# JuliaQuantumControl/GRAPE.jl

Measured on AMD Instinct MI355X. Metric: GRAPE gradient evals/sec (N=64, 1000 steps, 128 traj), higher is better.
Workload: dtype f64

## Files before the change

### grape.jl_amd/api.py

```python
from __future__ import annotations

import ctypes as C
import os
import subprocess
import sys

import numpy as np

_HERE = os.path.dirname(os.path.abspath(__file__))
_CSRC = os.path.join(_HERE, "csrc")
_LIBNAME = "libgrape_hip.so"

J_T_SM, J_T_SS, J_T_RE = 0, 1, 2
GRAD_GRADGEN, GRAD_TAYLOR = 0, 1
PROP_EXP, PROP_SERIES = 0, 1
ABI_VERSION = 7

STATUS = {0: "GRAPE_OK", -1: "GRAPE_ERR_INVALID", -2: "GRAPE_ERR_HIP", -3: "GRAPE_ERR_CHI_NORM",
          -4: "GRAPE_ERR_SINGULAR", -5: "GRAPE_ERR_TAYLOR", -6: "GRAPE_ERR_NO_CONTROLS", -7: "GRAPE_ERR_AGAIN",
          -8: "GRAPE_ERR_HOST"}

EXPORTS = ["grape_create", "grape_destroy", "grape_eval", "grape_forward", "grape_backward",
           "grape_forward_device", "grape_backward_device", "grape_check", "grape_get_propagator",
           "grape_get_tau_grads", "grape_get_storage", "grape_get_timings", "grape_reset_timings", "grape_get_work",
           "grape_last_error", "grape_abi_version", "grape_set_fused_sweeps", "grape_get_sums", "grape_backward_xi",
           "grape_get_final_states", "grape_backward_chi",
           "grape_get_time_gradient", "grape_set_tlist", "grape_eval_batch", "grape_get_batch_info", "grape_create_open",
           "grape_hvp", "grape_get_hvp_info", "grape_open_time_gradient", "grape_open_hvp", "grape_get_open_hvp_info",
           "grape_open_eval_batch", "grape_get_open_batch_info", "grape_open_set_running_cost", "grape_open_backward_xi"]


class GrapeHipError(RuntimeError):
    def __init__(self, code, msg):
        super().__init__(f"{STATUS.get(code, code)}: {msg}")
        self.code = code


class _Problem(C.Structure):
    _fields_ = [("abi_version", C.c_int32), ("N", C.c_int32), ("L", C.c_int32), ("K", C.c_int32),
# ... 39 lines not shown
                'grape_asm_co_start:\n\t.incbin "grape_asm.co"\ngrape_asm_co_end:\n\t.byte 0\n'
                '\t.section .note.GNU-stack,"",@progbits\n')
    cmds.append(["gcc", "-c", "-fPIC", "asm_embed.S", "-o", "asm_embed.o"])
    for c in cmds:
        res = subprocess.run(c, capture_output=True, text=True, cwd=work)
        if verbose or res.returncode:
            print(" ".join(c), res.stdout, res.stderr)
        if res.returncode:
            raise RuntimeError("assembling the gfx950 kernels failed")
    return emb_o


def _sources():
    srcs = [os.path.join(_CSRC, f) for f in ("grape_hip.hip", "grape_t18.hip", "grape_kernels.hip.h", "grape_large.hip.h",
                                             "grape_series.hip.h", "grape_cheby.hip.h", "grape_t18.hip.h", "grape_t18_coeffs.h",
                                             "grape_deriv3.hip.h", "grape_timegrad.hip.h", "grape_batch.hip.h", "grape_lindblad.hip.h", "grape_lindblad_tg.hip.h", "grape_hvp.hip.h", "grape_lindblad_hvp.hip.h", "grape_lindblad_batch.hip.h", "grape_lindblad_rc.hip.h", "grape_devmem.h", os.path.join("asm", "gen_t16.py"), os.path.join("asm", "gen_t16p.py"), os.path.join("asm", "gen_t18g.py"), os.path.join("asm", "gen_t18gp.py"), os.path.join("asm", "gen_d3.py"), os.path.join("asm", "gen_d3s.py"), os.path.join("asm", "gen_lg.py"), os.path.join("asm", "gen_d4.py"), os.path.join("asm", "gcn.py"))]
    return srcs, os.path.join(_HERE, "..", "include", "grape_hip.h")


def _up_to_date(out: str) -> bool:
    srcs, hdr = _sources()
    return os.path.exists(out) and all(os.path.getmtime(out) >= os.path.getmtime(s) for s in srcs + [hdr])


def build_library(force: bool = False, verbose: bool = False, extra_flags=(), out: str | None = None) -> str:
    import fcntl
    import shutil
    import tempfile
    out = out or library_path()
    if not force and _up_to_date(out):
        return out
# ... 55 lines not shown
    lib.grape_create.argtypes = [C.POINTER(vp), C.POINTER(_Problem)]
    lib.grape_create_open.argtypes = [C.POINTER(vp), C.POINTER(_Problem), C.POINTER(_Lindblad)]
    lib.grape_destroy.argtypes = [vp]
    lib.grape_destroy.restype = None
    lib.grape_eval.argtypes = [vp, vp, dp, vp, vp, vp]
    lib.grape_forward.argtypes = [vp, vp, vp]
    lib.grape_backward.argtypes = [vp, vp, vp]
    lib.grape_forward_device.argtypes = [vp, vp, vp, vp]
    lib.grape_backward_device.argtypes = [vp, vp, vp, vp]
    lib.grape_check.argtypes = [vp, vp]
    lib.grape_get_propagator.argtypes = [vp, ip, ip, vp]
    lib.grape_get_tau_grads.argtypes = [vp, vp]
    lib.grape_get_storage.argtypes = [vp, ip, vp]
    lib.grape_get_timings.argtypes = [vp, vp, ip]
    lib.grape_get_work.argtypes = [vp, vp, ip]
    lib.grape_reset_timings.argtypes = [vp]
    lib.grape_set_fused_sweeps.argtypes = [vp, ip]
    lib.grape_get_sums.argtypes = [vp, vp]
    lib.grape_get_final_states.argtypes = [vp, vp]
    lib.grape_backward_chi.argtypes = [vp, vp, vp]
    lib.grape_backward_xi.argtypes = [vp, vp, vp, vp, C.c_double, vp]
    lib.grape_get_time_gradient.argtypes = [vp, vp]
    lib.grape_open_time_gradient.argtypes = [vp, vp]
    lib.grape_set_tlist.argtypes = [vp, vp]
    lib.grape_eval_batch.argtypes = [vp, ip, vp, vp, vp, vp]
    lib.grape_get_batch_info.argtypes = [vp, vp, ip]
    lib.grape_hvp.argtypes = [vp, ip, vp, vp]
    lib.grape_get_hvp_info.argtypes = [vp, vp, ip]
    lib.grape_open_hvp.argtypes = [vp, ip, vp, vp]
    lib.grape_get_open_hvp_info.argtypes = [vp, vp, ip]
# ... 236 lines not shown

    def timings(self):
        ms = np.full(8, -1.0)
        self._lib.grape_get_timings(self._h, ms.ctypes.data, 8)
        out = dict(zip(["expm", "forward", "backward", "deriv", "reduce", "total"], ms[:6].tolist()))
        if ms[6] >= 0.0:
            out["host_enqueue"] = float(ms[6])
        if ms[7] >= 0.0:
            out["gradient_allreduce_us"] = float(ms[7]) * 1e3
        return out

    def reset_timings(self):
        self._chk(self._lib.grape_reset_timings(self._h))

    def work(self):
        w = np.zeros(19)
        self._lib.grape_get_work(self._h, w.ctypes.data, 19)
        return dict(cells=w[0], squarings=w[1], flop_expm=w[2], flop_deriv=w[3], deriv_orders=w[4],
                    pivoted_cells=w[5], expm_cells=w[6], series_terms=w[7], series_steps=w[8],
                    t18_mfma_flop=w[9], t18_squarings=w[10], t18_cells=w[11], matrix_free_fallback=w[12], t16_cells=w[13],
                    asm_kernel=w[14], asm_deriv_kernel=w[15], asm_blocked_products=w[16],
                    walk_steps=w[17], scan_block=w[18])


def liouvillian(H, cops=()):
    H = np.asarray(H, dtype=np.complex128)
    d = H.shape[0]
    if H.shape != (d, d):
        raise ValueError(f"H must be [d, d], got {H.shape}")
    eye = np.eye(d)
    heff = H.copy()
    for A in cops:
        A = np.asarray(A, dtype=np.complex128)
        heff = heff - 0.5j * (A.conj().T @ A)
    out = np.kron(eye, heff) - np.kron(heff.conj(), eye)
    for A in cops:
        A = np.asarray(A, dtype=np.complex128)
# ... 172 lines not shown
```

### grape.jl_amd/csrc/asm/gen_t16.py

```python
import os
import re
import struct
import sys

sys.path.insert(0, os.path.dirname(os.path.abspath(__file__)))
from gcn import Prog, Reg, V, A, S, VCC, EXEC, Neg, Abs, kernel_text

NT = 4
NP = 64
LDB = (3 * NP + 2) * 8
PLB = NP * 8
TROW = 16 * LDB
PLANES = NP * LDB
E1 = PLANES
EXH = 256 * 8 + 128
EXW = 2 * EXH
E2 = E1 + 4 * EXW
RED = E2 + 4 * EXW
XS0 = RED + 16 * 8
XS1 = XS0 + 1024
LDS_BYTES = XS1 + 1024
KERNARG = 136

HERE = os.path.dirname(os.path.abspath(__file__))


def t16_coeffs():
    txt = open(os.path.join(HERE, "..", "grape_t18_coeffs.h")).read()
    c = {}
    for m in re.finditer(r"#define\s+T16_(C\d+|THETA)\s+([-+0-9.eE]+)", txt):
        c[m.group(1)] = float(m.group(2))
    assert len(c) == 17, c
    return c


def dbits(x):
    b = struct.unpack("<Q", struct.pack("<d", x))[0]
# ... 335 lines not shown
        p.salu("s_lshl_b32", t0, t1, 16)
        p.salu("s_lshr_b32", t1, t1, 16)
        p.salu("s_add_u32", self.s_sb.sub(0), self.s_Sf.sub(0), t0)
        p.salu("s_addc_u32", self.s_sb.sub(1), self.s_Sf.sub(1), t1)

    def cell_bases_finish(self, kc):
        p = self.p
        t0, t1 = self.s_tmp[0], self.s_tmp[1]
        p.s_waitcnt(lgkm=0)
        p.s_cmp("s_cmp_lg_u64", self.s_rep, 0)
        p.salu("s_cselect_b32", self.s_k, self.s_k, kc)
        p.salu("s_lshl_b32", t0, self.s_k, 16)
        p.salu("s_lshr_b32", t1, self.s_k, 16)
        p.salu("s_add_u32", self.s_hb.sub(0), self.s_H0.sub(0), t0)
        p.salu("s_addc_u32", self.s_hb.sub(1), self.s_H0.sub(1), t1)
        p.salu("s_lshl_b32", t0, self.s_snext, 20)
        p.salu("s_sub_u32", self.s_dt.sub(1), self.s_dt.sub(1), t0)

    def cell_bases(self, kc, n, cell):
        self.cell_bases_issue(kc, n, cell)
        self.cell_bases_finish(kc)

    def fetch(self, u, dst, half=None):
        p = self.p
        (i0, j0), (i1, j1) = TILES[2 * u], TILES[2 * u + 1]
        toff = self.s_tmp[2]
        p.s_cmp("s_cmp_lt_u32", self.s_wave, 2)
        self.ssel(toff, (16 * i0 * NP + 16 * j0) * 8, (16 * i1 * NP + 16 * j1) * 8)
        if half in (None, 0):
            p.salu("s_add_u32", self.s_t0.sub(0), self.s_hb.sub(0), toff)
            p.salu("s_addc_u32", self.s_t0.sub(1), self.s_hb.sub(1), 0)
# ... 292 lines not shown
                streams.append([lambda xr=xr, ar_=ar_: self.acc_read(xr, ar_),
                                lambda xi=xi, ai_=ai_: self.acc_read(xi, ai_),
                                lambda xr=xr: p.valu("v_mul_f64", xr, c[2], xr),
                                lambda xi=xi: p.valu("v_mul_f64", xi, c[2], xi),
                                lambda xr=xr, a2r=a2r: p.valu("v_fma_f64", xr, c[1], a2r, xr),
                                lambda xi=xi, a2i=a2i: p.valu("v_fma_f64", xi, c[1], a2i, xi),
                                lambda xs=xs, xr=xr, xi=xi: p.valu("v_add_f64", xs, xr, xi),
                                lambda r=r, a2r=a2r, a2i=a2i: p.valu("v_add_f64", A2sm[sl].d(r), a2r, a2i)])
            self.interleave(streams)

        self.product(Qt, [A2re, A2im, A2sm], fused={"valu": valu2, "stores": lambda sl: self.plane_stores(sl, tt[0], tt[1], Qt[sl][1])})
        for t in tt + A2sm:
            vp.free(t)
        self.cell_bases_finish(self.s_nkc)
        self.stamp(3)
        facc, gacc, cacc = vp.alloc(), vp.alloc(), vp.alloc()
        for acc in (facc, gacc, cacc):
            for j in range(8):
                p.valu("v_mov_b32", acc.sub(j), 0)
        streams = []
        for sl in range(4):
            for r in range(4):
                k = len(streams) % 4
                p1, p2, p3 = (Qt[sl][j].d(r) for j in range(3))
                a2r, a2i = A2re[sl].d(r), A2im[sl].d(r)
                f, g_, cs = facc.d(k), gacc.d(k), cacc.d(k)
                streams.append([
                    lambda p3=p3, p1=p1: p.valu("v_add_f64", p3, p3, Neg(p1)),
                    lambda p1=p1, p2=p2: p.valu("v_add_f64", p1, p1, Neg(p2)),
                    lambda p3=p3, p2=p2: p.valu("v_add_f64", p3, p3, Neg(p2)),
# ... 2 lines not shown
                    lambda g_=g_, a2r=a2r, p1=p1: p.valu("v_fma_f64", g_, a2r, p1, g_),
                    lambda cs=cs, a2i=a2i: p.valu("v_add_f64", cs, cs, Abs(a2i)),
                    lambda f=f, p3=p3: p.valu("v_fma_f64", f, p3, p3, f),
                    lambda g_=g_, a2i=a2i, p3=p3: p.valu("v_fma_f64", g_, a2i, p3, g_)])
        for g in range(0, 16, 4):
            self.interleave(streams[g:g + 4])
        f, g_, cs = facc.d(0), gacc.d(0), cacc.d(0)
        for k in range(1, 4):
            p.valu("v_add_f64", f, f, facc.d(k))
            p.valu("v_add_f64", g_, g_, gacc.d(k))
            p.valu("v_add_f64", cs, cs, cacc.d(k))
        ones, ct = cacc.d(1), vp.alloc(1)
        lo, hi = dbits(1.0)
        p.valu("v_mov_b32", ones.sub(0), lo)
        p.valu("v_mov_b32", ones.sub(1), hi)
        p.mfma(ct, ones, cs, 0)
        tmp = cacc.d(2)
        self.wave_reduce(f, tmp, "v_add_f64")
        self.wave_reduce(g_, tmp, "v_add_f64")
        mx = cacc.d(3)
        p.valu("v_mov_b64", mx, ct.d(0))
        for ctrl in ("quad_perm:[1,0,3,2]", "quad_perm:[2,3,0,1]", "row_half_mirror", "row_mirror"):
            p.dpp_mov(tmp.sub(0), mx.sub(0), ctrl)
            p.dpp_mov(tmp.sub(1), mx.sub(1), ctrl)
            p.valu("v_max_f64", mx, mx, tmp)
        vrd = ct.sub(2)
        p.salu("s_lshl_b32", self.s_tmp[0], self.s_wave, 3)
        p.salu("s_add_u32", self.s_tmp[0], self.s_tmp[0], RED)
        p.valu("v_mov_b32", vrd, self.s_tmp[0])
        p.salu("s_mov_b64", self.s_save, EXEC)
        self.set_exec(0, 0x80000000)
# ... 37 lines not shown
        p.s_cmp("s_cmp_eq_u64", S(58, 2), 0)
        p.salu("s_cselect_b32", self.s_tmp[4], 2, 0)
        p.salu("s_or_b32", self.s_prop, self.s_prop, self.s_tmp[4])
        p.valu("v_cndmask_b32", vz.sub(1), 1, 0, S(58, 2))
        p.salu("s_lshl_b32", self.s_tmp[2], self.s_cell, 2)
        p.valu("v_mov_b32", vz.sub(2), self.s_tmp[2])
        p.salu("s_mov_b64", self.s_save, EXEC)
        p.s_cmp("s_cmp_eq_u32", self.s_wave, 0)
        p.salu("s_cselect_b32", self.s_tmp[4], 1, 0)
        p.salu("s_mov_b32", self.s_tmp[5], 0)
        p.salu("s_mov_b64", EXEC, S(self.s_tmp[4].idx, 2))
        p.global_store(1, vz.sub(2), vz.sub(1), self.s_verdict)
        p.salu("s_mov_b64", EXEC, self.s_save)
        for t in (vtf, vtg, vt2, vz):
            vp.free(t)
        self.A2p_re, self.A2p_im = ap.alloc(4), ap.alloc(4)
        Bre, Bim, Bsm = [None] * 4, [None] * 4, [None] * 4
        tt = [vp.alloc(), vp.alloc()]

        def valu3(sl):
            Bre[sl], Bim[sl], Bsm[sl] = vp.alloc(), vp.alloc(), vp.alloc()
            streams = []
            for r in range(4):
                y0r, xs, y0i = (Qt[sl][j].d(r) for j in range(3))
                a2r, a2i = A2re[sl].d(r), A2im[sl].d(r)
                xr, xi = tt[0].d(r), tt[1].d(r)
                br, bi, bs = Bre[sl].d(r), Bim[sl].d(r), Bsm[sl].d(r)
                ar_, ai_ = A_(sl, r)
                pr, pi_ = self.A2p_re.sub(8 * sl, 8).d(r), self.A2p_im.sub(8 * sl, 8).d(r)
                streams.append([
# ... 101 lines not shown
                            "after_first": lambda: bsm([0]), "post": post4})
        for t in tt:
            vp.free(t)
        if not self.early_free:
            ap.free(self.A2p_re)
            ap.free(self.A2p_im)
        for t in Bre + Bim + Bsm:
            vp.free(t)
        self.stamp(9)
        if not self.early_free:
            ap.free(self.As_re)
            ap.free(self.As_im)
        Un = vp.alloc(8, at=self.UT)
        uid = len(p.ins)
        L_sq, L_sq_loop, L_res = f"L_sq_{uid}", f"L_sq_loop_{uid}", f"L_res_{uid}"
        p.s_cmp("s_cmp_lg_u32", self.s_scur, 0)
        p.s_branch("s_cbranch_scc1", L_sq)
        streams = []
        for sl in range(4):
            for r in range(4):
                p1, p2, p3 = (Qt[sl][j].d(r) for j in range(3))
                ur, ui = Un.sub(16 * sl + 4 * r, 2), Un.sub(16 * sl + 4 * r + 2, 2)
                streams.append([lambda ur=ur, p1=p1, p2=p2: p.valu("v_add_f64", ur, p1, Neg(p2)),
                                lambda ui=ui, p3=p3, p1=p1: p.valu("v_add_f64", ui, p3, Neg(p1)),
                                lambda ui=ui, p2=p2: p.valu("v_add_f64", ui, ui, Neg(p2))])
        for g in range(0, 16, 4):
            self.interleave(streams[g:g + 4])
        p.s_barrier()
        p.s_branch("s_branch", L_res)
        p.label(L_sq)
        vp.free(Un)
        in_place_y(range(4))
        p.s_barrier()
        p.salu("s_mov_b32", self.s_sqc, self.s_scur)
        p.label(L_sq_loop)
        Q2 = [[vp.alloc() for _ in range(3)] for _ in range(4)]

        def valu_sq(sl):
            for r in range(4):
                p.valu("v_add_f64", Qt[sl][1].d(r), Qt[sl][0].d(r), Qt[sl][2].d(r))

        self.product(Q2, [[Qt[sl][0] for sl in range(4)], [Qt[sl][2] for sl in range(4)], [Qt[sl][1] for sl in range(4)]],
                     fused={"valu": valu_sq, "stores": lambda sl: self.plane_stores(sl, Qt[sl][0], Qt[sl][2], Qt[sl][1])})
        streams = []
        for sl in range(4):
            for r in range(4):
                q1, q2, q3 = (Q2[sl][j].d(r) for j in range(3))
                tr, ti = Qt[sl][0].d(r), Qt[sl][2].d(r)
                streams.append([lambda tr=tr, q1=q1, q2=q2: p.valu("v_add_f64", tr, q1, Neg(q2)),
# ... 315 lines not shown
```

### grape.jl_amd/csrc/grape_hip.hip

```cpp
#include "../../include/grape_hip.h"
#include "grape_kernels.hip.h"
#include "grape_t18_coeffs.h"
#include "grape_econ_coeffs.h"
#include "grape_large.hip.h"
#include "grape_series.hip.h"
#include "grape_cheby.hip.h"
#include "grape_timegrad.hip.h"
#include "grape_lindblad.hip.h"
#include "grape_lindblad_tg.hip.h"
#include "grape_hvp.hip.h"
#include "grape_lindblad_hvp.hip.h"
#include "grape_lindblad_batch.hip.h"
#include "grape_lindblad_rc.hip.h"
#include "grape_devmem.h"

#include <rccl/rccl.h>
#include <dlfcn.h>
#include <mutex>

#include <algorithm>
#include <chrono>
#include <cmath>
#include <cstdio>
#include <cstdlib>
#include <cstring>
#include <new>
#include <stdexcept>
#include <string>
#include <thread>
// ... 63 lines not shown
    double *d_eps = nullptr;
    double2 *d_U = nullptr, *d_fw = nullptr, *d_bw = nullptr, *d_tg = nullptr;
    double *d_ret = nullptr;
    double *d_out = nullptr;
    double *d_f = nullptr, *d_G = nullptr, *d_rho = nullptr;
    int *d_flags = nullptr;
    int *d_cellflag = nullptr;
    int KC = 0;
    bool herm = false;
    bool herm_ctrl = false;
    bool t18 = false;
    bool t18_small = true;
    bool t16 = true;
    double *d_gram = nullptr;
    int *d_celllist = nullptr;
    bool asm16 = false;
    bool asm16p = false;
    double *d_dte = nullptr;
    bool asm18gp = false;
    bool asm18g = false;
    int *d_wgtab = nullptr, *d_prog = nullptr, *d_splan = nullptr;
    double2 *d_xinit = nullptr;
    int asm_blocks = 0;
    int last_walk_fuse = 0;
    bool asm_sq = true;
    int asm_walk = 0;
    bool foreign_stream = false;
    bool credit_pending = false;
    std::vector<double> bal;
    std::vector<double> bal_stage_chi, bal_stage_xi;
// ... 2520 lines not shown
                    gram[(size_t)kc * GS + (size_t)a * M + b] = gram[(size_t)kc * GS + (size_t)b * M + a] = sum;
                }
        }
        if (!p->hc_per_traj)
            for (int l = 0; l < L; ++l) kap_shared[l] = shape_factor(p->Hc + (size_t)l * nn2, gram[(size_t)(1 + l) * M + (1 + l)]);
        parallel_for(KCn, [&](int kc) {
            const int k = repk[kc] < 0 ? kc : repk[kc];
            for (int a = 0; a < M; ++a) {
                const double fro2 = gram[(size_t)kc * GS + (size_t)a * M + a];
                const double *o = a == 0 ? p->H0 + (size_t)k * nn2 : p->Hc + ((size_t)(p->hc_per_traj ? k : 0) * L + (a - 1)) * nn2;
                gram[(size_t)kc * GS + (size_t)M * M + a] = (a > 0 && !p->hc_per_traj) ? kap_shared[a - 1] : shape_factor(o, fro2);
            }
        });
        CCHK(h->mem.alloc(&h->d_gram, gram.size()));
        CCHK(hipMemcpy(h->d_gram, gram.data(), gram.size() * 8, hipMemcpyHostToDevice));
    }
    if (h->large && h->series) {
        const int per_xcd = std::max(1, h->num_cus / 8), S = h->NP / 16;
        if (per_xcd < S) {
            h->err = "prop_method = GRAPE_PROP_SERIES with N > 64 needs NP / 16 co-resident workgroups per XCD";
            return fail(GRAPE_ERR_INVALID);
        }
        h->cheby_S = S;
        h->cheby_pair = h->fuse && per_xcd >= 2 * S;
        if (!h->cheby_pair) h->fuse = false;
        h->cheby_round = 8 * std::max(1, per_xcd / ((h->cheby_pair ? 2 : 1) * S));
        CCHK(h->mem.alloc(&h->d_xch, (size_t)2 * K * 4 * NP));
        CCHK(h->mem.alloc(&h->d_xcc, (size_t)2 * K * 32));
    }
    if (h->large && !h->series) {
// ... 95 lines not shown
                if (h->d_Sf) {
                    CtrlSumArgs ca{};
                    ca.Hcf = h->d_Hcf; ca.eps = h->d_eps; ca.shape = h->d_shape; ca.Sf = h->d_Sf;
                    ca.L = h->L; ca.N_T = h->N_T; ca.pp2 = 2 * h->NP * h->NP;
                    ca.per_traj = h->p.hc_per_traj ? 1 : 0; ca.rep = h->d_rep;
                    hipLaunchKernelGGL(ctrl_sum_kernel, dim3((unsigned)((ca.per_traj ? h->KC : 1) * h->N_T), std::max(1, ca.pp2 / 2 / 2048)), dim3(256), 0, s, ca);
                    HIPCHK(h, hipGetLastError());
                    ea.Sf = h->d_Sf;
                }
                const bool t16 = h->d_celllist != nullptr;
                ea.cell_list = h->d_celllist; ea.listed = 0;
                if (t16) {
                    T16PlanArgs pa{};
                    pa.gram = h->d_gram; pa.eps = h->d_eps; pa.shape = h->d_shape; pa.dts = h->d_dts; pa.flags = h->d_flags;
                    pa.KC = h->KC; pa.L = h->L; pa.N_T = h->N_T; pa.N = h->N;
                    pa.splan = (h->asm16 && h->asm_sq) ? h->d_splan : nullptr;
                    hipLaunchKernelGGL(t16_plan_kernel, dim3((unsigned)((ncell + 255) / 256)), dim3(256), 0, s, pa);
                    HIPCHK(h, hipGetLastError());
                }
                const int blocks16 = (t16 && h->NT == 3) ? 8 * (int)std::max<long>(1, std::min<long>((long)(h->num_cus / 8) * 2, (ncell + 7) / 8)) : t18_blocks;
                h->credit_pending = false;
                if (h->asm18g) {
                    walk_fuse = h->asm_walk & (1 | ((h->fuse && h->fuse_on && h->want_bw) ? 2 : 0));
                    if (walk_fuse) HIPCHK(h, hipMemsetAsync(h->d_prog, 0, (size_t)2 * h->K * sizeof(int), s));
                    const void *walk[6] = {h->d_wgtab, h->d_xinit, h->d_fw, h->d_bw, h->d_prog, h->d_splan};
                    if (h->asm18gp) {
                        hipLaunchKernelGGL(dte_kernel, dim3((unsigned)((h->N_T + 255) / 256)), dim3(256), 0, s, (const double *)h->d_eps,
                                           (const double *)h->d_shape, (const double *)h->d_dts, h->L, h->N_T, 2, h->d_dte);
                        HIPCHK(h, hipGetLastError());
                    }
                    e = (hipError_t)grape_t18g_asm_launch(&ea, sizeof(ea), h->d_cellflag, (void *)s, h->asm_blocks, walk, walk_fuse, h->K,
// ... 1044 lines not shown
    }
    HIPCHK(h, hipSetDevice(h->device));
    HIPCHK(h, hipDeviceSynchronize());
    for (auto &ring : h->ph)
        for (auto &p : ring) p.used = false;
    h->n_fwd = h->n_bwd = 0;
    h->n_eval = 0;
    return GRAPE_OK;
}
GRAPE_BARRIER(h ? &h->err : &g_create_error)

int grape_get_work(grape_handle *h, double *out, int n) try {
    if (!h || !out || n < 4) return GRAPE_ERR_INVALID;
    if (h->open) return open_work(h, out, n);
    if (!h->shards.empty()) {
        const int m = n < 19 ? n : 19;
        std::fill(out, out + m, 0.0);
        for (grape_handle *c : h->shards) {
            double cw[19] = {0.};
            const int rc = grape_get_work(c, cw, m);
            if (rc < 0) return multi_fail(h, c, rc);
            for (int i = 0; i < m; ++i) out[i] = (i == 15 || i == 16 || i == 18) ? cw[i] : out[i] + cw[i];
        }
        if (m > 14 && out[14] > 0.0) out[14] = h->shards[0]->asm16p ? 3.0 : h->shards[0]->asm18gp ? 4.0 : h->shards[0]->asm18g ? 2.0 : 1.0;
        return 4;
    }
    HIPCHK(h, hipSetDevice(h->device));
    HIPCHK(h, hipDeviceSynchronize());
    if (h->credit_pending) {
        ExpmArgs ea{};
        ea.H0f = h->d_H0f; ea.Hcf = h->d_Hcf; ea.eps = h->d_eps; ea.shape = h->d_shape; ea.dts = h->d_dts;
        ea.flags = h->d_flags; ea.stats = h->d_stats; ea.Sf = h->d_Sf;
        ea.K = h->KC; ea.rep = h->d_rep; ea.L = h->L; ea.N_T = h->N_T; ea.hc_per_traj = h->p.hc_per_traj;
        ea.n1 = h->d_n1; ea.n1_k = h->K;
// ... 34 lines not shown
    }
    if (n > 16) out[16] = (h->large && !h->series && h->t18 && h->lg_asm) ? 1.0 : 0.0;
    if (n > 17) {
        double carried = 0.0;
        if (h->last_walk_fuse && h->d_prog) {
            std::vector<int> prog((size_t)2 * h->K);
            HIPCHK(h, hipMemcpy(prog.data(), h->d_prog, prog.size() * sizeof(int), hipMemcpyDeviceToHost));
            for (int k = 0; k < h->K; ++k) {
                if (h->last_walk_fuse & 1) carried += prog[(size_t)k];
                if (h->last_walk_fuse & 2) carried += prog[(size_t)h->K + k];
            }
        }
        out[17] = carried;
    }
    if (n > 18) out[18] = h->scan16 ? (double)h->scan_Bk : 0.0;
    return 4;
}
GRAPE_BARRIER(h ? &h->err : &g_create_error)

int grape_get_time_gradient(grape_handle *h, double *dJdt) try {
    if (h && h->open) return open_refuse(h, "grape_get_time_gradient");
    if (!h || !dJdt) return GRAPE_ERR_INVALID;
    const int N_T = h->N_T;
    if (!h->shards.empty()) {
        std::vector<double> part((size_t)N_T);
        for (size_t g = 0; g < h->shards.size(); ++g) {
            const int rc = grape_get_time_gradient(h->shards[g], g == 0 ? dJdt : part.data());
            if (rc) return multi_fail(h, h->shards[g], rc);
            if (g > 0) for (int n = 0; n < N_T; ++n) dJdt[n] += part[n];
        }
        return GRAPE_OK;
// ... 533 lines not shown
```

### grape.jl_amd/csrc/grape_kernels.hip.h

```cpp
#pragma once
#include <hip/hip_runtime.h>
#include <stdint.h>

typedef double d4 __attribute__((ext_vector_type(4)));

#define MFMA64(a, b, c) __builtin_amdgcn_mfma_f64_16x16x4f64((a), (b), (c), 0, 0, 0)

__device__ __constant__ double c_pade3[4] = {120., 60., 12., 1.};
__device__ __constant__ double c_pade5[6] = {30240., 15120., 3360., 420., 30., 1.};
__device__ __constant__ double c_pade7[8] = {17297280., 8648640., 1995840., 277200., 25200., 1512., 56., 1.};
__device__ __constant__ double c_pade9[10] = {17643225600., 8821612800., 2075673600., 302702400.,
                                              30270240., 2162160., 110880., 3960., 90., 1.};
#define B13_0 64764752532480000.
#define B13_1 32382376266240000.
#define B13_2 7771770303897600.
#define B13_3 1187353796428800.
#define B13_4 129060195264000.
#define B13_5 10559470521600.
#define B13_6 670442572800.
#define B13_7 33522128640.
#define B13_8 1323241920.
#define B13_9 40840800.
#define B13_10 960960.
#define B13_11 16380.
// ... 26 lines not shown
#ifdef GRAPE_DIAG
    int ablate;
    unsigned long long *stamps;
#endif
};

#define T16_PLAN_R 1.15
#define T16_PLAN_RS 1.11
#define T16_PLAN_SMAX 3
struct T16PlanArgs {
    const double *gram;
    const double *eps, *shape, *dts;
    int *flags;
    int KC, L, N_T, N;
    int *splan;
};
__global__ void __launch_bounds__(256) t16_plan_kernel(T16PlanArgs a) {
    const int cell = blockIdx.x * 256 + threadIdx.x;
    bool out = false;
    if (cell < a.KC * a.N_T) {
        const int kc = cell / a.N_T, n = cell - kc * a.N_T, M = a.L + 1;
        const double *G = a.gram + (size_t)kc * (M * M + M), *kap = G + M * M;
        double e[9];
        e[0] = 1.0;
        for (int l = 0; l < a.L; ++l) e[1 + l] = a.eps[(size_t)l * a.N_T + n] * (a.shape ? a.shape[(size_t)l * a.N_T + n] : 1.0);
        double m2 = 0., wk = 0., w = 0.;
        for (int i = 0; i < M; ++i) {
            for (int j = 0; j < M; ++j) m2 += e[i] * e[j] * G[i * M + j];
            const double wi = fabs(e[i]) * sqrt(fmax(G[i * M + i], 0.0));
            w += wi; wk += wi * kap[i];
        }
        const double dt = a.dts[n];
        const double r = 2.0 * fabs(dt) * sqrt(fmax(m2, 0.0) / (double)a.N) * (w > 0.0 ? wk / w : 1.0);
        out = !(r <= T16_PLAN_R);
        if (a.splan) {
            int sq = 0;
            if (out) {
                double rs = r;
                while (sq < T16_PLAN_SMAX && !(rs <= T16_PLAN_RS)) { rs *= 0.5; ++sq; }
                out = !(rs <= T16_PLAN_RS);
                if (out) sq = 0;
            }
            a.splan[cell] = sq;
        }
    }
    const unsigned long long m = __ballot(out);
    if ((threadIdx.x & 63) == 0 && m) atomicAdd(&a.flags[6], (int)__popcll(m));
}
__device__ __forceinline__ bool t16_skipped(const int *flags, const int ncell) { return 4L * flags[6] > (long)ncell; }

struct CtrlSumArgs {
    const double *Hcf, *eps, *shape;
    double *Sf;
    int L, N_T, pp2;
    int per_traj;
    const int *rep;
};
__device__ __forceinline__ void ctrl_sum_body(CtrlSumArgs a) {
// ... 2855 lines not shown
    int deg0, deg1;
    int *batch_econ;
};
__global__ void deriv_econ_kernel(DerivEconArgs a) {
    const int batch = blockIdx.x * blockDim.x + threadIdx.x;
    if (batch >= a.nbatch_total) return;
    const int k = batch / a.batches_per_k, n0 = (batch - k * a.batches_per_k) * 16;
    const int kc = a.cls ? a.cls[k] : k;
    bool ok = a.cell_deg || !t16_skipped(a.flags, a.KC * a.N_T);
    int deg = 0;
    for (int n = n0; ok && n < min(n0 + 16, a.N_T); ++n) {
        const int cell = kc * a.N_T + n;
        int d;
        if (a.cell_deg) d = a.cell_deg[cell];
        else {
            const int sq = a.splan ? a.splan[cell] : 0;
            d = a.verdict[cell] != 0 ? 0 : sq == 0 ? a.deg0 : sq == 1 ? a.deg1 : 0;
        }
        ok = d > 0;
        deg = max(deg, d);
    }
    a.batch_econ[batch] = ok ? deg : 0;
}

struct DerivSubArgs {
    DerivMfmaArgs m;
    const double *rb;
    int rb_k;
    double sub_theta;
    const int *batch_flag;
};
// ... 662 lines not shown
```

### grape.jl_amd/csrc/grape_t18.hip

```cpp
#include <hip/hip_runtime.h>
#include <stdint.h>
#include <string.h>
#include <type_traits>
#include <mutex>
#include <vector>
#include <stdlib.h>
#include <stdio.h>
namespace {
#include "grape_t18.hip.h"
#define GRAPE_BATCH_T18_UNIT
#include "grape_batch.hip.h"
#include "grape_deriv3.hip.h"
#include "grape_econ_coeffs.h"

template <int NT, bool SYM, bool CHEB, bool T16 = false>
hipError_t launch(const ExpmArgs &a, hipStream_t s, int blocks) {
    static size_t lds_set[64] = {0};
    const size_t lds = sizeof(double) * (size_t)T18Lds<NT>::TOTAL;
    int dev = 0;
    hipGetDevice(&dev);
    if (lds_set[dev & 63] < lds) {
        hipError_t e = hipFuncSetAttribute((const void *)expm_t18_kernel<NT, SYM, CHEB, T16>, hipFuncAttributeMaxDynamicSharedMemorySize, (int)lds);
        if (e != hipSuccess) return e;
        lds_set[dev & 63] = lds;
// ... 107 lines not shown
__global__ void __launch_bounds__(256) t16_post_kernel(ExpmArgs a, const int *verdict, const int *prog, int nprog, const int *splan) {
    const int tid = threadIdx.x, lane = tid & 63, ncell = a.K * a.N_T;
    if (t16_skipped(a.flags, ncell)) return;
    if (prog && blockIdx.x == 0) {
        unsigned long long steps = 0;
        for (int i = tid; i < nprog; i += 256) steps += (unsigned long long)prog[i];
        for (int off = 32; off >= 1; off >>= 1) steps += __shfl_xor(steps, off, 64);
        if (lane == 0 && steps) stat_add(a.stats, 12, steps * 4ull * 2ull);
    }
    const int cell = blockIdx.x * 256 + tid;
    const bool valid = cell < ncell;
    const bool ok = valid && verdict[cell] == 0;
    if (valid && !ok) a.cell_list[atomicAdd(&a.flags[4], 1)] = cell;
    const unsigned long long m_ok = __ballot(ok), m_valid = __ballot(valid);
    {
        unsigned long long sq = valid ? (unsigned long long)splan[cell] : 0ull;
        unsigned long long sq_ok = ok ? sq : 0ull;
        for (int off = 32; off >= 1; off >>= 1) { sq += __shfl_xor(sq, off, 64); sq_ok += __shfl_xor(sq_ok, off, 64); }
        if (lane == 0 && sq) stat_add(a.stats, 12, sq * 4ull * 192ull);
        if (lane == 0 && sq_ok) stat_add(a.stats, 13, sq_ok);
    }
    if (lane == 0 && m_valid) {
        stat_add(a.stats, 12, (unsigned long long)__popcll(m_valid) * 4ull * (unsigned long long)(T16Count<4>::CELL + 1));
        if (m_ok) {
            stat_add(a.stats, 14, (unsigned long long)__popcll(m_ok));
            stat_add(a.stats, 15, (unsigned long long)__popcll(m_ok));
        }
        atomicAdd(&a.flags[5], (int)__popcll(m_valid));
    }
}

// ... 434 lines not shown
```

### include/grape_hip.h

```cpp
#ifndef GRAPE_HIP_H
#define GRAPE_HIP_H

#include <stddef.h>
#include <stdint.h>

#ifdef __cplusplus
extern "C" {
#endif

#define GRAPE_HIP_ABI_VERSION 7

typedef struct grape_handle grape_handle;

typedef enum {
    GRAPE_OK = 0,
    GRAPE_ERR_INVALID = -1,
    GRAPE_ERR_HIP = -2,
    GRAPE_ERR_CHI_NORM = -3,
    GRAPE_ERR_SINGULAR = -4,
    GRAPE_ERR_TAYLOR = -5,
    GRAPE_ERR_NO_CONTROLS = -6,
    GRAPE_ERR_AGAIN = -7,
    GRAPE_ERR_HOST = -8
} grape_status;
// ... 74 lines not shown
int grape_backward_device(grape_handle *h, const double *d_f, double *d_G, void *stream);

int grape_set_fused_sweeps(grape_handle *h, int on);

int grape_check(grape_handle *h, void *stream);

int grape_get_propagator(grape_handle *h, int k, int n, double *out);

int grape_get_tau_grads(grape_handle *h, double *out );
int grape_get_storage(grape_handle *h, int which , double *out );

int grape_get_timings(grape_handle *h, double *ms, int n);
int grape_reset_timings(grape_handle *h);
int grape_get_work(grape_handle *h, double *out, int n);

int grape_get_time_gradient(grape_handle *h, double *dJdt );

int grape_open_time_gradient(grape_handle *h, double *dJdt );

int grape_set_tlist(grape_handle *h, const double *tlist );

int grape_eval_batch(grape_handle *h, int P, const double *pulsevals, double *J, double *G, double *tau);

int grape_get_batch_info(grape_handle *h, double *out, int n);

int grape_hvp(grape_handle *h, int nv, const double *V, double *HV);

int grape_get_hvp_info(grape_handle *h, double *out, int n);

int grape_open_hvp(grape_handle *h, int nv, const double *V, double *HV);
// ... 20 lines not shown
```

Baseline: 54.13.

## Certify T16 expm truncation a priori via precomputed trace polynomial tables

Precomputes, at handle creation, per-trajectory-class trace tables of products of H0/Hc powers, so the plan kernel can bound the norm of the eighth power of the generator as a polynomial in the pulse amplitudes. Cells that pass this bound get a CERT bit in the squaring plan. The asm T16 kernel then skips its in-kernel residual verification reductions for those cells, and the verdict flag is cleared ahead of time. The cost is extra setup work, a per-cell polynomial evaluation in the planner, and reliance on the correctness of the certified bound.

New measurement: 54.82 (median of 6 runs). +1.3%, better.

```diff
diff --git a/grape.jl_amd/api.py b/grape.jl_amd/api.py
--- a/grape.jl_amd/api.py
+++ b/grape.jl_amd/api.py
@@ -22,7 +22,7 @@
 
 EXPORTS = ["grape_create", "grape_destroy", "grape_eval", "grape_forward", "grape_backward",
            "grape_forward_device", "grape_backward_device", "grape_check", "grape_get_propagator",
-           "grape_get_tau_grads", "grape_get_storage", "grape_get_timings", "grape_reset_timings", "grape_get_work",
+           "grape_get_tau_grads", "grape_get_storage", "grape_get_timings", "grape_reset_timings", "grape_get_work", "grape_get_cert_table",
            "grape_last_error", "grape_abi_version", "grape_set_fused_sweeps", "grape_get_sums", "grape_backward_xi",
            "grape_get_final_states", "grape_backward_chi",
            "grape_get_time_gradient", "grape_set_tlist", "grape_eval_batch", "grape_get_batch_info", "grape_create_open",
@@ -92,7 +92,7 @@
 def _sources():
     srcs = [os.path.join(_CSRC, f) for f in ("grape_hip.hip", "grape_t18.hip", "grape_kernels.hip.h", "grape_large.hip.h",
                                              "grape_series.hip.h", "grape_cheby.hip.h", "grape_t18.hip.h", "grape_t18_coeffs.h",
-                                             "grape_deriv3.hip.h", "grape_timegrad.hip.h", "grape_batch.hip.h", "grape_lindblad.hip.h", "grape_lindblad_tg.hip.h", "grape_hvp.hip.h", "grape_lindblad_hvp.hip.h", "grape_lindblad_batch.hip.h", "grape_lindblad_rc.hip.h", "grape_devmem.h", os.path.join("asm", "gen_t16.py"), os.path.join("asm", "gen_t16p.py"), os.path.join("asm", "gen_t18g.py"), os.path.join("asm", "gen_t18gp.py"), os.path.join("asm", "gen_d3.py"), os.path.join("asm", "gen_d3s.py"), os.path.join("asm", "gen_lg.py"), os.path.join("asm", "gen_d4.py"), os.path.join("asm", "gcn.py"))]
+                                             "grape_deriv3.hip.h", "grape_timegrad.hip.h", "grape_batch.hip.h", "grape_lindblad.hip.h", "grape_lindblad_tg.hip.h", "grape_hvp.hip.h", "grape_lindblad_hvp.hip.h", "grape_lindblad_batch.hip.h", "grape_lindblad_rc.hip.h", "grape_devmem.h", "grape_cert.hip.h", os.path.join("asm", "gen_t16.py"), os.path.join("asm", "gen_t16p.py"), os.path.join("asm", "gen_t18g.py"), os.path.join("asm", "gen_t18gp.py"), os.path.join("asm", "gen_d3.py"), os.path.join("asm", "gen_d3s.py"), os.path.join("asm", "gen_lg.py"), os.path.join("asm", "gen_d4.py"), os.path.join("asm", "gcn.py"))]
     return srcs, os.path.join(_HERE, "..", "include", "grape_hip.h")
 
 
@@ -178,6 +178,7 @@
     lib.grape_get_storage.argtypes = [vp, ip, vp]
     lib.grape_get_timings.argtypes = [vp, vp, ip]
     lib.grape_get_work.argtypes = [vp, vp, ip]
+    lib.grape_get_cert_table.argtypes = [vp, vp, vp, vp]
     lib.grape_reset_timings.argtypes = [vp]
     lib.grape_set_fused_sweeps.argtypes = [vp, ip]
     lib.grape_get_sums.argtypes = [vp, vp]
@@ -444,13 +445,23 @@
         self._chk(self._lib.grape_reset_timings(self._h))
 
     def work(self):
-        w = np.zeros(19)
-        self._lib.grape_get_work(self._h, w.ctypes.data, 19)
+        w = np.zeros(20)
+        self._lib.grape_get_work(self._h, w.ctypes.data, 20)
         return dict(cells=w[0], squarings=w[1], flop_expm=w[2], flop_deriv=w[3], deriv_orders=w[4],
                     pivoted_cells=w[5], expm_cells=w[6], series_terms=w[7], series_steps=w[8],
                     t18_mfma_flop=w[9], t18_squarings=w[10], t18_cells=w[11], matrix_free_fallback=w[12], t16_cells=w[13],
                     asm_kernel=w[14], asm_deriv_kernel=w[15], asm_blocked_products=w[16],
-                    walk_steps=w[17], scan_block=w[18])
+                    walk_steps=w[17], scan_block=w[18], t16_certified=w[19])
+
+    def cert_table(self):
+        dims = np.zeros(3, np.int32)
+        self._chk(self._lib.grape_get_cert_table(self._h, dims.ctypes.data, None, None))
+        KC, n8, n6 = (int(x) for x in dims)
+        coef, exps = np.zeros((KC, n8 + n6)), np.zeros(n8 + n6, np.int32)
+        if n8 + n6:
+            self._chk(self._lib.grape_get_cert_table(self._h, dims.ctypes.data, coef.ctypes.data, exps.ctypes.data))
+        ex = np.stack([(exps >> (4 * l)) & 15 for l in range(self.L)], axis=1) if n8 + n6 else np.zeros((0, self.L), np.int32)
+        return coef[:, :n8], coef[:, n8:], ex
 
 
 def liouvillian(H, cops=()):
diff --git a/grape.jl_amd/csrc/asm/gen_t16.py b/grape.jl_amd/csrc/asm/gen_t16.py
--- a/grape.jl_amd/csrc/asm/gen_t16.py
+++ b/grape.jl_amd/csrc/asm/gen_t16.py
@@ -5,6 +5,7 @@
 
 sys.path.insert(0, os.path.dirname(os.path.abspath(__file__)))
 from gcn import Prog, Reg, V, A, S, VCC, EXEC, Neg, Abs, kernel_text
+from gcn import HZ_MFMA_TO_VALU as gcn_wait_valu, HZ_MFMA_TO_MEM as gcn_wait_mem
 
 NT = 4
 NP = 64
@@ -21,6 +22,8 @@
 XS1 = XS0 + 1024
 LDS_BYTES = XS1 + 1024
 KERNARG = 136
+SQ_MASK = 0xFF
+CERT_BIT = 0x100
 
 HERE = os.path.dirname(os.path.abspath(__file__))
 
@@ -386,7 +389,8 @@
         p.salu("s_lshr_b32", t1, self.s_k, 16)
         p.salu("s_add_u32", self.s_hb.sub(0), self.s_H0.sub(0), t0)
         p.salu("s_addc_u32", self.s_hb.sub(1), self.s_H0.sub(1), t1)
-        p.salu("s_lshl_b32", t0, self.s_snext, 20)
+        p.salu("s_and_b32", t0, self.s_snext, SQ_MASK)
+        p.salu("s_lshl_b32", t0, t0, 20)
         p.salu("s_sub_u32", self.s_dt.sub(1), self.s_dt.sub(1), t0)
 
     def cell_bases(self, kc, n, cell):
@@ -709,6 +713,10 @@
             vp.free(t)
         self.cell_bases_finish(self.s_nkc)
         self.stamp(3)
+        uid = len(p.ins)
+        L_cert, L_cert2, L_ones, L_vdone = f"L_cert_{uid}", f"L_cert2_{uid}", f"L_ones_{uid}", f"L_vdone_{uid}"
+        p.salu("s_and_b32", self.s_tmp[0], self.s_scur, CERT_BIT)
+        p.s_branch("s_cbranch_scc1", L_cert)
         facc, gacc, cacc = vp.alloc(), vp.alloc(), vp.alloc()
         for acc in (facc, gacc, cacc):
             for j in range(8):
@@ -741,7 +749,10 @@
         lo, hi = dbits(1.0)
         p.valu("v_mov_b32", ones.sub(0), lo)
         p.valu("v_mov_b32", ones.sub(1), hi)
+        p.label(L_ones)
         p.mfma(ct, ones, cs, 0)
+        p.salu("s_and_b32", self.s_tmp[0], self.s_scur, CERT_BIT)
+        p.s_branch("s_cbranch_scc1", L_cert2)
         tmp = cacc.d(2)
         self.wave_reduce(f, tmp, "v_add_f64")
         self.wave_reduce(g_, tmp, "v_add_f64")
@@ -809,6 +820,17 @@
         p.salu("s_mov_b64", EXEC, self.s_save)
         for t in (vtf, vtg, vt2, vz):
             vp.free(t)
+        p.s_branch("s_branch", L_vdone)
+        p.label(L_cert)
+        p.nop(gcn_wait_valu)
+        in_place_y(range(4))
+        p.s_branch("s_branch", L_ones)
+        p.label(L_cert2)
+        p.nop(gcn_wait_mem)
+        p.s_waitcnt(lgkm=0)
+        p.s_barrier()
+        p.salu("s_and_b32", self.s_prop, self.s_prop, 1)
+        p.label(L_vdone)
         self.A2p_re, self.A2p_im = ap.alloc(4), ap.alloc(4)
         Bre, Bim, Bsm = [None] * 4, [None] * 4, [None] * 4
         tt = [vp.alloc(), vp.alloc()]
@@ -940,7 +962,7 @@
         Un = vp.alloc(8, at=self.UT)
         uid = len(p.ins)
         L_sq, L_sq_loop, L_res = f"L_sq_{uid}", f"L_sq_loop_{uid}", f"L_res_{uid}"
-        p.s_cmp("s_cmp_lg_u32", self.s_scur, 0)
+        p.salu("s_and_b32", self.s_tmp[0], self.s_scur, SQ_MASK)
         p.s_branch("s_cbranch_scc1", L_sq)
         streams = []
         for sl in range(4):
@@ -958,7 +980,7 @@
         vp.free(Un)
         in_place_y(range(4))
         p.s_barrier()
-        p.salu("s_mov_b32", self.s_sqc, self.s_scur)
+        p.salu("s_and_b32", self.s_sqc, self.s_scur, SQ_MASK)
         p.label(L_sq_loop)
         Q2 = [[vp.alloc() for _ in range(3)] for _ in range(4)]
 
diff --git a/grape.jl_amd/csrc/grape_cert.hip.h b/grape.jl_amd/csrc/grape_cert.hip.h
--- /dev/null
+++ b/grape.jl_amd/csrc/grape_cert.hip.h
@@ -0,0 +1,123 @@
+#pragma once
+
+#include <hip/hip_runtime.h>
+
+#include <cstdint>
+#include <map>
+#include <vector>
+
+#define GRAPE_CERT_LMAX 4
+
+struct CertMonomials {
+    std::vector<uint32_t> key;
+    std::map<uint32_t, int> index;
+    CertMonomials(int M, int d) {
+        gen(M, d, 0, 0u);
+        for (size_t i = 0; i < key.size(); ++i) index[key[i]] = (int)i;
+    }
+    int size() const { return (int)key.size(); }
+
+private:
+    void gen(int M, int left, int a, uint32_t k) {
+        if (a == M - 1) { key.push_back(k | ((uint32_t)left << (4 * a))); return; }
+        for (int e = left; e >= 0; --e) gen(M, left - e, a + 1, k | ((uint32_t)e << (4 * a)));
+    }
+};
+
+struct CertJobs {
+    std::vector<int> row, pair;
+    void from(const std::vector<std::vector<int>> &lists) {
+        row.assign(1, 0);
+        pair.clear();
+        for (const auto &l : lists) {
+            pair.insert(pair.end(), l.begin(), l.end());
+            row.push_back((int)pair.size() / 2);
+        }
+    }
+};
+
+struct CertPlan {
+    int M, n2, n3, n4, n6, n8, nmat;
+    CertJobs mm2, mm34, tr;
+    std::vector<int> exps;
+    explicit CertPlan(int L) {
+        M = L + 1;
+        const CertMonomials m2(M, 2), m3(M, 3), m4(M, 4), m6(M, 6), m8(M, 8);
+        n2 = m2.size(); n3 = m3.size(); n4 = m4.size(); n6 = m6.size(); n8 = m8.size();
+        const int o2 = M, o3 = o2 + n2, o4 = o3 + n3;
+        nmat = o4 + n4;
+        auto var = [&](int a) { return (uint32_t)1 << (4 * a); };
+        std::vector<std::vector<int>> l2(n2), l34(n3 + n4), lt(n8 + n6);
+        for (int a = 0; a < M; ++a)
+            for (int b = 0; b < M; ++b) { auto &l = l2[m2.index.at(var(a) + var(b))]; l.push_back(a); l.push_back(b); }
+        for (int i = 0; i < n2; ++i)
+            for (int c = 0; c < M; ++c) { auto &l = l34[m3.index.at(m2.key[i] + var(c))]; l.push_back(o2 + i); l.push_back(c); }
+        for (int i = 0; i < n2; ++i)
+            for (int j = 0; j < n2; ++j) { auto &l = l34[n3 + m4.index.at(m2.key[i] + m2.key[j])]; l.push_back(o2 + i); l.push_back(o2 + j); }
+        for (int i = 0; i < n4; ++i)
+            for (int j = 0; j < n4; ++j) { auto &l = lt[m8.index.at(m4.key[i] + m4.key[j])]; l.push_back(o4 + i); l.push_back(o4 + j); }
+        for (int i = 0; i < n3; ++i)
+            for (int j = 0; j < n3; ++j) { auto &l = lt[n8 + m6.index.at(m3.key[i] + m3.key[j])]; l.push_back(o3 + i); l.push_back(o3 + j); }
+        mm2.from(l2); mm34.from(l34); tr.from(lt);
+        for (int i = 0; i < n8; ++i) exps.push_back((int)(m8.key[i] >> 4));
+        for (int i = 0; i < n6; ++i) exps.push_back((int)(m6.key[i] >> 4));
+    }
+};
+
+__global__ void __launch_bounds__(256) cert_load_kernel(const double *H0f, const double *Hcf, const int *rep, int kc0, int hc_per_traj, int L,
+                                                        int N, int NP, int nmat, double2 *scratch) {
+    const int a = blockIdx.x, c = blockIdx.y, kc = kc0 + c, k = rep ? rep[kc] : kc;
+    const size_t pp = (size_t)NP * NP;
+    const double *src = a == 0 ? H0f + (size_t)k * 2 * pp : Hcf + ((size_t)(hc_per_traj ? k : 0) * L + (a - 1)) * 2 * pp;
+    double2 *dst = scratch + ((size_t)c * nmat + a) * N * N;
+    for (int e = threadIdx.x; e < N * N; e += 256) {
+        const int i = e / N, j = e - i * N;
+        dst[e] = make_double2(src[(size_t)i * NP + j], src[pp + (size_t)i * NP + j]);
+    }
+}
+
+__global__ void __launch_bounds__(256) cert_mm_kernel(double2 *scratch, int nmat, int N, int dst0, const int *row, const int *pair) {
+    double2 *base = scratch + (size_t)blockIdx.y * nmat * N * N;
+    double2 *dst = base + (size_t)(dst0 + blockIdx.x) * N * N;
+    const int p0 = row[blockIdx.x], p1 = row[blockIdx.x + 1];
+    for (int e = threadIdx.x; e < N * N; e += 256) {
+        const int i = e / N, j = e - i * N;
+        double sr = 0., si = 0.;
+        for (int q = p0; q < p1; ++q) {
+            const double2 *A = base + (size_t)pair[2 * q] * N * N + (size_t)i * N, *B = base + (size_t)pair[2 * q + 1] * N * N + j;
+            double tr = 0., ti = 0.;
+            for (int k = 0; k < N; ++k) {
+                const double2 x = A[k], y = B[(size_t)k * N];
+                tr += x.x * y.x - x.y * y.y;
+                ti += x.x * y.y + x.y * y.x;
+            }
+            sr += tr; si += ti;
+        }
+        dst[e] = make_double2(sr, si);
+    }
+}
+
+__global__ void __launch_bounds__(256) cert_trace_kernel(const double2 *scratch, int nmat, int N, const int *row, const int *pair, int nt,
+                                                         double *table) {
+    __shared__ double red[256];
+    const double2 *base = scratch + (size_t)blockIdx.y * nmat * N * N;
+    const int p0 = row[blockIdx.x], p1 = row[blockIdx.x + 1];
+    double sum = 0.;
+    for (int q = p0; q < p1; ++q) {
+        const double2 *A = base + (size_t)pair[2 * q] * N * N, *B = base + (size_t)pair[2 * q + 1] * N * N;
+        double t = 0.;
+        for (int e = threadIdx.x; e < N * N; e += 256) {
+            const int i = e / N, j = e - i * N;
+            const double2 x = A[e], y = B[(size_t)j * N + i];
+            t += x.x * y.x - x.y * y.y;
+        }
+        sum += t;
+    }
+    red[threadIdx.x] = sum;
+    __syncthreads();
+    for (int off = 128; off >= 1; off >>= 1) {
+        if ((int)threadIdx.x < off) red[threadIdx.x] += red[threadIdx.x + off];
+        __syncthreads();
+    }
+    if (threadIdx.x == 0) table[(size_t)blockIdx.y * nt + blockIdx.x] = red[0];
+}
diff --git a/grape.jl_amd/csrc/grape_hip.hip b/grape.jl_amd/csrc/grape_hip.hip
--- a/grape.jl_amd/csrc/grape_hip.hip
+++ b/grape.jl_amd/csrc/grape_hip.hip
@@ -13,6 +13,7 @@
 #include "grape_lindblad_batch.hip.h"
 #include "grape_lindblad_rc.hip.h"
 #include "grape_devmem.h"
+#include "grape_cert.hip.h"
 
 #include <rccl/rccl.h>
 #include <dlfcn.h>
@@ -106,6 +107,9 @@
     bool t16 = true;
     double *d_gram = nullptr;
     int *d_celllist = nullptr;
+    double *d_cert = nullptr;
+    int *d_cert_exp = nullptr;
+    int cert_n8 = 0, cert_n6 = 0;
     bool asm16 = false;
     bool asm16p = false;
     double *d_dte = nullptr;
@@ -2656,6 +2660,38 @@
         });
         CCHK(h->mem.alloc(&h->d_gram, gram.size()));
         CCHK(hipMemcpy(h->d_gram, gram.data(), gram.size() * 8, hipMemcpyHostToDevice));
+        const char *envc = getenv("GRAPE_EXPM_CERT");
+        if (h->asm16 && L >= 1 && L <= GRAPE_CERT_LMAX && !(envc && atoi(envc) == 0)) {
+            const CertPlan pl(L);
+            const int nt = pl.n8 + pl.n6;
+            h->cert_n8 = pl.n8; h->cert_n6 = pl.n6;
+            CCHK(h->mem.alloc(&h->d_cert, (size_t)KCn * nt));
+            CCHK(h->mem.alloc(&h->d_cert_exp, (size_t)nt));
+            CCHK(hipMemcpy(h->d_cert_exp, pl.exps.data(), (size_t)nt * sizeof(int), hipMemcpyHostToDevice));
+            DeviceBufs tmp;
+            int *d_job[6] = {nullptr, nullptr, nullptr, nullptr, nullptr, nullptr};
+            const std::vector<int> *job[6] = {&pl.mm2.row, &pl.mm2.pair, &pl.mm34.row, &pl.mm34.pair, &pl.tr.row, &pl.tr.pair};
+            for (int i = 0; i < 6; ++i) {
+                CCHK(tmp.alloc(&d_job[i], job[i]->size()));
+                CCHK(hipMemcpy(d_job[i], job[i]->data(), job[i]->size() * sizeof(int), hipMemcpyHostToDevice));
+            }
+            const size_t per_class = (size_t)pl.nmat * N * N;
+            const int chunk = (int)std::max<size_t>(1, std::min<size_t>((size_t)KCn, ((size_t)64 << 20) / (per_class * sizeof(double2))));
+            double2 *d_scr = nullptr;
+            CCHK(tmp.alloc(&d_scr, per_class * chunk));
+            for (int kc0 = 0; kc0 < KCn; kc0 += chunk) {
+                const unsigned nc = (unsigned)std::min(chunk, KCn - kc0);
+                hipLaunchKernelGGL(cert_load_kernel, dim3((unsigned)pl.M, nc), dim3(256), 0, 0, (const double *)h->d_H0f, (const double *)h->d_Hcf,
+                                   (const int *)h->d_rep, kc0, p->hc_per_traj ? 1 : 0, L, N, NP, pl.nmat, d_scr);
+                hipLaunchKernelGGL(cert_mm_kernel, dim3((unsigned)pl.n2, nc), dim3(256), 0, 0, d_scr, pl.nmat, N, pl.M, (const int *)d_job[0], (const int *)d_job[1]);
+                hipLaunchKernelGGL(cert_mm_kernel, dim3((unsigned)(pl.n3 + pl.n4), nc), dim3(256), 0, 0, d_scr, pl.nmat, N, pl.M + pl.n2, (const int *)d_job[2],
+                                   (const int *)d_job[3]);
+                hipLaunchKernelGGL(cert_trace_kernel, dim3((unsigned)nt, nc), dim3(256), 0, 0, (const double2 *)d_scr, pl.nmat, N, (const int *)d_job[4],
+                                   (const int *)d_job[5], nt, h->d_cert + (size_t)kc0 * nt);
+                CCHK(hipGetLastError());
+            }
+            CCHK(hipDeviceSynchronize());
+        }
     }
     if (h->large && h->series) {
         const int per_xcd = std::max(1, h->num_cus / 8), S = h->NP / 16;
@@ -2781,7 +2817,10 @@
                     T16PlanArgs pa{};
                     pa.gram = h->d_gram; pa.eps = h->d_eps; pa.shape = h->d_shape; pa.dts = h->d_dts; pa.flags = h->d_flags;
                     pa.KC = h->KC; pa.L = h->L; pa.N_T = h->N_T; pa.N = h->N;
-                    pa.splan = (h->asm16 && h->asm_sq) ? h->d_splan : nullptr;
+                    pa.splan = (h->asm16 && (h->asm_sq || h->d_cert)) ? h->d_splan : nullptr;
+                    pa.sq_on = h->asm_sq ? 1 : 0;
+                    pa.cert = h->d_cert; pa.cert_exp = h->d_cert_exp; pa.n8 = h->cert_n8; pa.n6 = h->cert_n6;
+                    pa.verdict = h->d_cellflag;
                     hipLaunchKernelGGL(t16_plan_kernel, dim3((unsigned)((ncell + 255) / 256)), dim3(256), 0, s, pa);
                     HIPCHK(h, hipGetLastError());
                 }
@@ -3856,10 +3895,10 @@
     if (!h || !out || n < 4) return GRAPE_ERR_INVALID;
     if (h->open) return open_work(h, out, n);
     if (!h->shards.empty()) {
-        const int m = n < 19 ? n : 19;
+        const int m = n < 20 ? n : 20;
         std::fill(out, out + m, 0.0);
         for (grape_handle *c : h->shards) {
-            double cw[19] = {0.};
+            double cw[20] = {0.};
             const int rc = grape_get_work(c, cw, m);
             if (rc < 0) return multi_fail(h, c, rc);
             for (int i = 0; i < m; ++i) out[i] = (i == 15 || i == 16 || i == 18) ? cw[i] : out[i] + cw[i];
@@ -3924,7 +3963,36 @@
         out[17] = carried;
     }
     if (n > 18) out[18] = h->scan16 ? (double)h->scan_Bk : 0.0;
+    if (n > 19) {
+        double certified = 0.0;
+        if (h->d_cert && h->d_splan && !h->series) {
+            const size_t ncell = (size_t)h->KC * h->N_T;
+            std::vector<int> plan(ncell);
+            int fl[8];
+            HIPCHK(h, hipMemcpy(plan.data(), h->d_splan, ncell * sizeof(int), hipMemcpyDeviceToHost));
+            HIPCHK(h, hipMemcpy(fl, h->d_flags, sizeof(fl), hipMemcpyDeviceToHost));
+            if (!(4L * fl[6] > (long)ncell))
+                for (int w : plan) certified += (w & T16_PLAN_CERT) ? 1.0 : 0.0;
+        }
+        out[19] = certified;
+    }
     return 4;
+}
+GRAPE_BARRIER(h ? &h->err : &g_create_error)
+
+int grape_get_cert_table(grape_handle *h, int *dims, double *coef, int *exps) try {
+    if (!h || !dims) return GRAPE_ERR_INVALID;
+    if (h->open || !h->shards.empty()) {
+        h->err = "grape_get_cert_table: a closed handle on one device";
+        return GRAPE_ERR_INVALID;
+    }
+    const int nt = h->cert_n8 + h->cert_n6;
+    dims[0] = h->KC; dims[1] = h->cert_n8; dims[2] = h->cert_n6;
+    if (!h->d_cert || !nt) { dims[1] = dims[2] = 0; return GRAPE_OK; }
+    HIPCHK(h, hipSetDevice(h->device));
+    if (coef) HIPCHK(h, hipMemcpy(coef, h->d_cert, (size_t)h->KC * nt * sizeof(double), hipMemcpyDeviceToHost));
+    if (exps) HIPCHK(h, hipMemcpy(exps, h->d_cert_exp, (size_t)nt * sizeof(int), hipMemcpyDeviceToHost));
+    return GRAPE_OK;
 }
 GRAPE_BARRIER(h ? &h->err : &g_create_error)
 
diff --git a/grape.jl_amd/csrc/grape_kernels.hip.h b/grape.jl_amd/csrc/grape_kernels.hip.h
--- a/grape.jl_amd/csrc/grape_kernels.hip.h
+++ b/grape.jl_amd/csrc/grape_kernels.hip.h
@@ -1,6 +1,8 @@
 #pragma once
 #include <hip/hip_runtime.h>
 #include <stdint.h>
+
+#include "grape_t18_coeffs.h"
 
 typedef double d4 __attribute__((ext_vector_type(4)));
 
@@ -64,7 +66,31 @@
     int *flags;
     int KC, L, N_T, N;
     int *splan;
+    int sq_on;
+    const double *cert;
+    const int *cert_exp;
+    int n8, n6;
+    int *verdict;
 };
+#define T16_PLAN_SQ_MASK 0xFF
+#define T16_PLAN_CERT 0x100
+__device__ __forceinline__ bool t16_certified(const double *t, const int *ex, const int n8, const int n6, const int L, const double *e,
+                                              const double dt, const int sq) {
+    double p[2] = {0., 0.}, S8 = 0.;
+    for (int i = 0; i < n8 + n6; ++i) {
+        unsigned x = (unsigned)ex[i];
+        double mono = 1.0;
+        for (int l = 0; l < L; ++l, x >>= 4)
+            for (unsigned q = x & 15u; q > 0; --q) mono *= e[l];
+        const double c = t[i];
+        p[i < n8 ? 0 : 1] += c * mono;
+        if (i < n8) S8 += fabs(c) * fabs(mono);
+    }
+    const double dt2 = dt * dt, dt8 = (dt2 * dt2) * (dt2 * dt2);
+    constexpr double th2 = T16_THETA * T16_THETA, th8 = (th2 * th2) * (th2 * th2);
+    const double lhs = (p[0] + 0x1p-30 * S8) * dt8 * (1.0 + 1e-6), rhs = ldexp(th8, 8 * sq);
+    return lhs <= rhs && p[1] >= 0.0;
+}
 __global__ void __launch_bounds__(256) t16_plan_kernel(T16PlanArgs a) {
     const int cell = blockIdx.x * 256 + threadIdx.x;
     bool out = false;
@@ -85,13 +111,15 @@
         out = !(r <= T16_PLAN_R);
         if (a.splan) {
             int sq = 0;
-            if (out) {
+            if (out && a.sq_on) {
                 double rs = r;
                 while (sq < T16_PLAN_SMAX && !(rs <= T16_PLAN_RS)) { rs *= 0.5; ++sq; }
                 out = !(rs <= T16_PLAN_RS);
                 if (out) sq = 0;
             }
-            a.splan[cell] = sq;
+            const bool cert = a.cert && t16_certified(a.cert + (size_t)kc * (a.n8 + a.n6), a.cert_exp, a.n8, a.n6, a.L, e + 1, dt, sq);
+            if (cert) a.verdict[cell] = 0;
+            a.splan[cell] = sq | (cert ? T16_PLAN_CERT : 0);
         }
     }
     const unsigned long long m = __ballot(out);
@@ -2977,7 +3005,7 @@
         int d;
         if (a.cell_deg) d = a.cell_deg[cell];
         else {
-            const int sq = a.splan ? a.splan[cell] : 0;
+            const int sq = a.splan ? (a.splan[cell] & T16_PLAN_SQ_MASK) : 0;
             d = a.verdict[cell] != 0 ? 0 : sq == 0 ? a.deg0 : sq == 1 ? a.deg1 : 0;
         }
         ok = d > 0;
diff --git a/grape.jl_amd/csrc/grape_t18.hip b/grape.jl_amd/csrc/grape_t18.hip
--- a/grape.jl_amd/csrc/grape_t18.hip
+++ b/grape.jl_amd/csrc/grape_t18.hip
@@ -145,7 +145,7 @@
     if (valid && !ok) a.cell_list[atomicAdd(&a.flags[4], 1)] = cell;
     const unsigned long long m_ok = __ballot(ok), m_valid = __ballot(valid);
     {
-        unsigned long long sq = valid ? (unsigned long long)splan[cell] : 0ull;
+        unsigned long long sq = valid ? (unsigned long long)(splan[cell] & T16_PLAN_SQ_MASK) : 0ull;
         unsigned long long sq_ok = ok ? sq : 0ull;
         for (int off = 32; off >= 1; off >>= 1) { sq += __shfl_xor(sq, off, 64); sq_ok += __shfl_xor(sq_ok, off, 64); }
         if (lane == 0 && sq) stat_add(a.stats, 12, sq * 4ull * 192ull);
diff --git a/include/grape_hip.h b/include/grape_hip.h
--- a/include/grape_hip.h
+++ b/include/grape_hip.h
@@ -112,6 +112,8 @@
 int grape_reset_timings(grape_handle *h);
 int grape_get_work(grape_handle *h, double *out, int n);
 
+int grape_get_cert_table(grape_handle *h, int *dims, double *coef, int *exps);
+
 int grape_get_time_gradient(grape_handle *h, double *dJdt );
 
 int grape_open_time_gradient(grape_handle *h, double *dJdt );
```
